# Luigi940260/orb-slam2-optimized

Hardware: AMD Instinct MI355X
Metric: RANSAC hypotheses/sec (EPnP relocalization batch, 2k corrs x 64 candidates) (higher is better)
Workload: dtype f64; 1 GPU; config 2 reloc_pnp: candidates x correspondences, iterate(300), exhaustive (40% inliers); candidates=64, candidates_per_gpu=64, correspondences=2000, hypotheses_per_candidate=300, params=SetRansacParameters(0.99,10,300,4,0.5,5.991)

## Files before the change

### orb-slam2-optimized_amd/csrc/kernels.hip

```cpp
#include <hip/hip_runtime.h>
#include <climits>

#ifndef RSC_REFINE_STAMPS
#define RSC_REFINE_STAMPS 0
#endif
namespace rsc {
__device__ uint64_t g_refine_stamps[64][24];
}
#ifndef RSC_SOLVE_STAMPS
#define RSC_SOLVE_STAMPS 0
#endif
namespace rsc {
__device__ uint64_t g_solve_stamps[3][4096][8];
}
#if RSC_SOLVE_STAMPS
#define RSC_JSVD_STAMP(k, j)                                                                           \
    do {                                                                                               \
        if (blockIdx.x < 4096 && (threadIdx.x & 63) == 0 && blockDim.x == 64) {                       \
            ::rsc::g_solve_stamps[2][blockIdx.x][j] = wall_clock64();                                  \
            ::rsc::g_solve_stamps[2][blockIdx.x][3] = (k);                                             \
        }                                                                                              \
    } while (0)
#define RSC_SOLVE_STAMP(st, k)                                                                         \
    do {                                                                                               \
// ... 12 lines not shown
#include "rsc_quad.h"
#include "rsc_math.h"
#include "rsc_kernels.h"

namespace rsc {

template <int NS>
__global__ __launch_bounds__(64) void pnp_eig_group_kernel(const DevPnP* __restrict__ probs,
                                                          const LaunchProb* __restrict__ lps,
                                                          const int2* __restrict__ wg_table,
                                                          const uint32_t* __restrict__ rng_T,
                                                          double* __restrict__ stage, int32_t* __restrict__ samples) {
    __shared__ __attribute__((aligned(16))) double smem[kEigHyps * kQuadRegion];
    pnp_eig_group_body<NS, 99, kEigLanes, kEigHyps>(probs, lps, wg_table, rng_T, stage, samples, smem);
}

template <int NS>
__global__ __launch_bounds__(128 * kSplitUnits) __attribute__((amdgpu_waves_per_eu(2))) void pnp_eig_split_kernel(
    const DevPnP* __restrict__ probs, const LaunchProb* __restrict__ lps, const int2* __restrict__ wg_table,
    int nwg_table, const uint32_t* __restrict__ rng_T, double* __restrict__ stage, int32_t* __restrict__ samples,
    unsigned* fault) {
    __shared__ __attribute__((aligned(16))) double smem[kSplitHyps * kQuadRegion];
    __shared__ __attribute__((aligned(16))) double dsub[kSplitHyps * kSplitDsub];
    __shared__ int pub[kSplitUnits], ack[kSplitUnits];
    pnp_eig_split_body<NS>(probs, lps, wg_table, nwg_table, rng_T, stage, samples, smem, dsub, pub, ack, fault);
}

template <int NS>
__global__ __launch_bounds__(64) void pnp_betas_kernel(const DevPnP* __restrict__ probs,
                                                       const LaunchProb* __restrict__ lps,
                                                       const int2* __restrict__ wg_table, int ngroups,
                                                       const double* __restrict__ stage,
                                                       const int32_t* __restrict__ samples,
                                                       float* __restrict__ poses, double* __restrict__ berr,
                                                       float* __restrict__ bpose, unsigned* __restrict__ bctr,
                                                       size_t hcap, int hb) {
    __shared__ __attribute__((aligned(16))) double smem[kBetasWaveSmemDoubles];
    pnp_betas_wave_body<NS>(probs, lps, wg_table, ngroups, hb, stage, samples, poses, berr, bpose, bctr, hcap, smem);
}

typedef float rsc_f2 __attribute__((ext_vector_type(2)));
__device__ __forceinline__ void pnp_inlier2(const float (&R)[9], const float (&t)[3], double fx, double fy, double cx,
                                            double cy, rsc_f2 X, rsc_f2 Y, rsc_f2 Z, rsc_f2 u, rsc_f2 v, rsc_f2 maxErr,
                                            bool& in0, bool& in1, bool& ok) {
    const rsc_f2 Xc = (R[0] * X + (R[1] * Y + R[2] * Z)) + t[0];
    const rsc_f2 Yc = (R[3] * X + (R[4] * Y + R[5] * Z)) + t[1];
    const rsc_f2 Zc = (R[6] * X + (R[7] * Y + R[8] * Z)) + t[2];
    const rsc_f2 r0 = {__builtin_amdgcn_rcpf(Zc.x), __builtin_amdgcn_rcpf(Zc.y)};
    const rsc_f2 e = __builtin_elementwise_fma(-Zc, r0, (rsc_f2){1.0f, 1.0f});
    const rsc_f2 iz = __builtin_elementwise_fma(e, r0, r0);
    const float a0 = fabsf(Zc.x), a1 = fabsf(Zc.y);
    ok = ok & (a0 >= 0x1p-126f) & (a0 <= 0x1p125f) & (a1 >= 0x1p-126f) & (a1 <= 0x1p125f);
    const rsc_f2 ue = {(float)(cx + fx * (double)Xc.x * (double)iz.x), (float)(cx + fx * (double)Xc.y * (double)iz.y)};
    const rsc_f2 ve = {(float)(cy + fy * (double)Yc.x * (double)iz.x), (float)(cy + fy * (double)Yc.y * (double)iz.y)};
    const rsc_f2 du = ue - u, dv = ve - v;
    const rsc_f2 e2 = du * du + dv * dv;
    in0 = e2.x < maxErr.x;
    in1 = e2.y < maxErr.y;
}

template <int PPT>
__global__ __launch_bounds__(256) void pnp_scan_kernel(const DevPnP* __restrict__ probs,
                                                       const LaunchProb* __restrict__ lps,
                                                       const int4* __restrict__ wg_table,
                                                       const float* __restrict__ poses,
                                                       int32_t* __restrict__ counts,
                                                       int32_t* __restrict__ counts_dev,
                                                       uint64_t* __restrict__ masks, int mask_words,
                                                       int32_t* __restrict__ qual) {
    constexpr int B = PPT <= 8 ? 64 : 512 / PPT;
    __shared__ int wave_cnt[4][B];
    __shared__ uint64_t mbuf[B][4][PPT];
    const int tid = threadIdx.x, lane = tid & 63, wave = tid >> 6;
    const int4 wt = wg_table[blockIdx.x];
    const LaunchProb& lp = lps[wt.x];
    const DevPnP& P = probs[lp.prob];
    const double fx = P.fx, fy = P.fy, cx = P.cx, cy = P.cy;
    float X[PPT], Y[PPT], Z[PPT], U[PPT], V[PPT], E[PPT];
    RSC_UNROLL for (int s = 0; s < PPT; ++s) {
        const int i = s * 256 + tid;
        if (i < P.n) {
            const float4 p = P.pts[i];
            const float2 q = P.uv[i];
            X[s] = p.x; Y[s] = p.y; Z[s] = p.z; E[s] = p.w * P.th2; U[s] = q.x; V[s] = q.y;
        } else {
            X[s] = 0.f; Y[s] = 0.f; Z[s] = 1.f; E[s] = -1.f; U[s] = 0.f; V[s] = 0.f;
        }
    }
    const float* pp = poses + (size_t)(lp.out0 + wt.y) * 12;
    float Rn[9], tn[3];
    RSC_UNROLL for (int k = 0; k < 9; ++k) Rn[k] = pp[k];
    RSC_UNROLL for (int k = 0; k < 3; ++k) tn[k] = pp[9 + k];
    for (int j = 0; j < wt.z; ++j) {
        float R[9], t[3];
        RSC_UNROLL for (int k = 0; k < 9; ++k) R[k] = Rn[k];
        RSC_UNROLL for (int k = 0; k < 3; ++k) t[k] = tn[k];
        if (j + 1 < wt.z) {
            pp += 12;
            RSC_UNROLL for (int k = 0; k < 9; ++k) Rn[k] = pp[k];
            RSC_UNROLL for (int k = 0; k < 3; ++k) tn[k] = pp[9 + k];
        }
        uint64_t b[PPT];
        if constexpr (PPT >= 2) {
            bool ok = true;
            RSC_UNROLL for (int s = 0; s < PPT; s += 2) {
                bool i0, i1;
                pnp_inlier2(R, t, fx, fy, cx, cy, (rsc_f2){X[s], X[s + 1]}, (rsc_f2){Y[s], Y[s + 1]},
                            (rsc_f2){Z[s], Z[s + 1]}, (rsc_f2){U[s], U[s + 1]}, (rsc_f2){V[s], V[s + 1]},
                            (rsc_f2){E[s], E[s + 1]}, i0, i1, ok);
                b[s] = __ballot(i0);
                b[s + 1] = __ballot(i1);
            }
            if (__builtin_expect(__any(!ok), 0)) {
                RSC_UNROLL for (int s = 0; s < PPT; ++s)
                    b[s] = __ballot(pnp_inlier(R, t, fx, fy, cx, cy, X[s], Y[s], Z[s], U[s], V[s], E[s]));
            }
        } else {
            RSC_UNROLL for (int s = 0; s < PPT; ++s)
                b[s] = __ballot(pnp_inlier(R, t, fx, fy, cx, cy, X[s], Y[s], Z[s], U[s], V[s], E[s]));
        }
        int cnt = 0;
        uint64_t mine = 0;
        RSC_UNROLL for (int s = 0; s < PPT; ++s) {
            cnt += __popcll(b[s]);
            mine = (lane == s) ? b[s] : mine;
        }
        const int jb = j % B;
        if (lane < PPT) mbuf[jb][wave][lane] = mine;
        if (lane == 0) wave_cnt[wave][jb] = cnt;
        if (jb == B - 1 || j == wt.z - 1) {
            __syncthreads();
// ... 758 lines not shown
    if (count <= 0) return hipSuccess;
    sim3_pick_kernel<<<count, 256, 0, st>>>(lps, counts, poses, pick);
    return hipGetLastError();
}

hipError_t launch_gather_records(const float* src, int stride, int take, const int32_t* idx, int n, float* dst,
                                 hipStream_t st) {
    if (n <= 0) return hipSuccess;
    gather_records_kernel<<<(n * take + 255) / 256, 256, 0, st>>>(src, stride, take, idx, n, dst);
    return hipGetLastError();
}

__global__ void rng_stream_kernel(const uint32_t* __restrict__ T, Window31 w, int g0, int n, int32_t* __restrict__ out) {
    const int i = blockIdx.x * blockDim.x + threadIdx.x;
    if (i >= n) return;
    uint32_t ww[31];
    RSC_UNROLL for (int j = 0; j < 31; ++j) ww[j] = w.w[j];
    out[i] = (int32_t)(rng_word(T, ww, g0 + i) >> 1);
}

template <int N>
static hipError_t launch_eig_rows(int nwgE, const int2* wgtE, const DevPnP* probs, const LaunchProb* lps,
                                  const uint32_t* T, double* stage, int32_t* samples, hipStream_t st) {
    if constexpr (kEigHyps == 4 * kRowsGroups) {
        pnp_eig_rows_kernel<N><<<nwgE, 256, 0, st>>>(probs, lps, wgtE, T, stage, samples);
        return hipSuccess;
    } else {
        return hipErrorInvalidValue;
    }
}

hipError_t launch_pnp_solve_split(int ns, int nwgE, const int2* wgtE, int nwgB, const int2* wgtB,
                                  const DevPnP* probs, const LaunchProb* lps, const uint32_t* T, double* stage,
                                  float* poses, int32_t* samples, const BetasScratch& bs, hipStream_t st,
                                  hipEvent_t eig_begin, hipEvent_t eig_end, bool eig_rows, bool eig_split,
                                  unsigned* fault, int betas_hb) {
    if (ns < 4 || ns > 6 || betas_hb < 1 || betas_hb > kBetasHyps) return hipErrorInvalidValue;
    if (eig_split && !eig_rows && !fault) return hipErrorInvalidValue;
    if (eig_begin) (void)hipEventRecord(eig_begin, st);
    switch (ns) {
#define RSC_CASE(N)                                                                                   \
    case N:                                                                                           \
        if (eig_rows) {                                                                               \
            const hipError_t e = launch_eig_rows<N>(nwgE, wgtE, probs, lps, T, stage, samples, st);   \
            if (e != hipSuccess) return e;                                                            \
        } else if (eig_split)                                                                         \
            pnp_eig_split_kernel<N><<<(nwgE + kSplitUnits - 1) / kSplitUnits, 128 * kSplitUnits, 0, st>>>( \
                probs, lps, wgtE, nwgE, T, stage, samples, fault);                                    \
        else                                                                                          \
            pnp_eig_group_kernel<N><<<nwgE, 64, 0, st>>>(probs, lps, wgtE, T, stage, samples);        \
        if (eig_end) (void)hipEventRecord(eig_end, st);                                               \
        pnp_betas_kernel<N><<<3 * nwgB, 64, 0, st>>>(probs, lps, wgtB, nwgB, stage, samples, poses,   \
                                                     bs.err, bs.pose, bs.ctr, bs.hcap, betas_hb);     \
        break;
        RSC_CASE(4) RSC_CASE(5) RSC_CASE(6)
#undef RSC_CASE
        default: return hipErrorInvalidValue;
    }
    return hipGetLastError();
}

__global__ __launch_bounds__(256) void selftest_math_kernel(int fn, const double* __restrict__ x, int n,
                                                            double* __restrict__ out) {
    const int i = blockIdx.x * 256 + threadIdx.x;
    if (i >= n) return;
    const double v = x[i];
    double r;
    switch (fn) {
        case 0: r = dm::sin(v); break;
        case 1: r = dm::cos(v); break;
        case 2: r = dm::acos(v); break;
        case 3: r = dm::cbrt(v); break;
        case 4: r = dm::log(v); break;
        case 5: r = (double)dm::logf((float)v); break;
        case 6: r = sqrt_unit(v); break;
        case 7: r = recip_unit(v); break;
        case 11: r = dm::pow_1_3(v); break;
        case 12: r = dm::pow_3_2(v); break;
        case 13: {
            const float z = (float)v;
            const float r0 = __builtin_amdgcn_rcpf(z);
            r = (double)__builtin_fmaf(__builtin_fmaf(-z, r0, 1.0f), r0, r0);
            break;
        }

        default: {
// ... 52 lines not shown
    copy_bytes_kernel<<<blocks, 256, 0, st>>>(static_cast<const uint8_t*>(src), static_cast<uint8_t*>(dst), n, unit);
    return hipGetLastError();
}

__global__ __launch_bounds__(64) void signal_kernel(uint32_t* flag, uint32_t v) {
    if (threadIdx.x == 0) __hip_atomic_store(flag, v, __ATOMIC_RELEASE, __HIP_MEMORY_SCOPE_SYSTEM);
}

hipError_t launch_signal(uint32_t* host_flag, uint32_t value, hipStream_t st) {
    signal_kernel<<<1, 64, 0, st>>>(host_flag, value);
    return hipGetLastError();
}

hipError_t launch_upload16(const void* host_src, void* dev_dst, size_t n16, hipStream_t st) {
    if (n16 == 0) return hipSuccess;
    const unsigned blocks = (unsigned)((n16 + 255) / 256);
    upload16_kernel<<<blocks, 256, 0, st>>>(static_cast<const uint4*>(host_src), static_cast<uint4*>(dev_dst), n16);
    return hipGetLastError();
}

hipError_t launch_selftest_math(int fn, const double* x, int n, double* out, hipStream_t st) {
    if (fn < 0 || fn > 13 || n <= 0) return hipErrorInvalidValue;
    if (fn == 10) {
        if (n % 34) return hipErrorInvalidValue;
        const int nrec = n / 34;
        selftest_qr_kernel<<<(nrec + 255) / 256, 256, 0, st>>>(x, nrec, out);
        return hipGetLastError();
    }
    selftest_math_kernel<<<(n + 255) / 256, 256, 0, st>>>(fn, x, n, out);
    return hipGetLastError();
}

hipError_t launch_pnp_scan(int ppt, int nwg, const DevPnP* probs, const LaunchProb* lps, const int4* wgt,
                           const float* poses, int32_t* counts, int32_t* counts_dev, uint64_t* masks, int mask_words,
                           int32_t* qual, hipStream_t st) {
    switch (ppt) {
#define RSC_CASE(P) case P: pnp_scan_kernel<P><<<nwg, 256, 0, st>>>(probs, lps, wgt, poses, counts, counts_dev, masks, mask_words, qual); break;
        RSC_CASE(1) RSC_CASE(2) RSC_CASE(4) RSC_CASE(8) RSC_CASE(16) RSC_CASE(32)
#undef RSC_CASE
        default: return hipErrorInvalidValue;
    }
    return hipGetLastError();
}

hipError_t read_solve_stamps(uint64_t* out) {
    return hipMemcpyFromSymbol(out, HIP_SYMBOL(g_solve_stamps), sizeof(uint64_t) * 3 * 4096 * 8, 0, hipMemcpyDeviceToHost);
}

hipError_t read_refine_stamps(uint64_t* out) {
    return hipMemcpyFromSymbol(out, HIP_SYMBOL(g_refine_stamps), sizeof(uint64_t) * 64 * 24, 0, hipMemcpyDeviceToHost);
}

hipError_t launch_pnp_refine(int njobs, const DevPnP* probs, const RefineJob* jobs, unsigned* fault, hipStream_t st) {
    if (!fault) return hipErrorInvalidValue;
    pnp_refine_kernel<<<njobs, 256, 0, st>>>(probs, jobs, fault);
    return hipGetLastError();
}

hipError_t launch_pnp_select_refine(int nsel, const DevPnP* probs, const RefineSel* sels, const int32_t* counts,
                                    uint64_t* masks, int mask_words, const float* poses, RefineSelOut* out,
                                    unsigned* fault, hipStream_t st) {
    if (nsel <= 0) return hipSuccess;
    if (!fault) return hipErrorInvalidValue;
    pnp_select_refine_kernel<<<nsel, 256, 0, st>>>(probs, sels, counts, masks, mask_words, poses, out, fault);
    return hipGetLastError();
}

hipError_t launch_sim3_solve(int nwg, const DevSim3* probs, const LaunchProb* lps, const int2* wgt, const uint32_t* T,
                             float* poses, int32_t* samples, hipStream_t st) {
    sim3_solve_kernel<<<nwg, 64, 0, st>>>(probs, lps, wgt, T, poses, samples);
    return hipGetLastError();
}

hipError_t launch_sim3_scan(int ppt, int nwg, const DevSim3* probs, const LaunchProb* lps, const int4* wgt,
                            const float* poses, int32_t* counts, int32_t* counts_dev, uint64_t* masks, int mask_words,
// ... 19 lines not shown
```

### orb-slam2-optimized_amd/csrc/rsc_api.cpp

```cpp
#include <hip/hip_runtime.h>
#include <cstdio>
#include <cstdlib>
#include <algorithm>
#include <array>
#include <chrono>
#include <cmath>
#include <cstring>
#include <string>
#include <vector>
#include <memory>
#include "../../include/rsc.h"
#include "rsc_kernels.h"
#include "rsc_engine.h"
#include "rsc_poseopt.h"
#include "rsc_sim3opt.h"
#include "rsc_orbmatch.h"
#include "rsc_sim3match.h"
#include "rsc_frameproj.h"
#include "rsc_kfproj.h"
#include "rsc_localproj.h"
#include "rsc_sim3compose.h"
#include "rsc_kfdb.h"
#include "rsc_bowvoc.h"

// ... 73 lines not shown
    rb.clear();
    for (size_t i = 0; i < n; ++i)
        if (i == 0 || prob_of(src[i]) != prob_of(src[i - 1])) rb.push_back(i);
    rb.push_back(n);
    size_t left[X] = {};
    for (int x = 0; x < X; ++x) runs[x].clear();
    for (size_t r = 0; r + 1 < rb.size(); ++r) {
        int best = 0;
        for (int x = 1; x < X; ++x) if (left[x] < left[best]) best = x;
        runs[best].push_back((int)r);
        left[best] += rb[r + 1] - rb[r];
    }
    size_t cr[X] = {}, cp[X] = {};
    for (size_t b = 0; b < n; ++b) {
        int x = (int)(b % X);
        if (!left[x])
            for (int y = 0; y < X; ++y) if (left[y] > left[x]) x = y;
        const int r = runs[x][cr[x]];
        wgs[b] = src[rb[r] + cp[x]];
        if (++cp[x] == rb[r + 1] - rb[r]) { cp[x] = 0; ++cr[x]; }
        --left[x];
    }
}

int scan_chunk(int total_hyps) {
    static const int target = [] {
        const char* m = std::getenv("RSC_SCAN_WGS");
        return m ? std::max(1, std::atoi(m)) : 2048;
    }();
    int hc = 32;
    while (hc > 8 && (total_hyps + hc - 1) / hc < target) hc >>= 1;
    return hc;
}

int ppt_for(int n) {
    int need = (n + 255) / 256;
    int p = 1;
    while (p < need) p <<= 1;
    return p;
}

}

constexpr int kSoCoopCUs = 256;
constexpr int kFaultWord = 4;

struct rsc_context {
    int device = 0;
    hipStream_t stream = nullptr;
    bool own_stream = false;
    RngTable table;
    DevBuf<uint32_t> d_table;
    DevBuf<float> d_poses;
    DevBuf<int32_t> d_counts;
    DevBuf<uint64_t> d_masks;
    DevBuf<int32_t> d_samples;
    DevBuf<double> d_stage;
    DevBuf<double> d_berr;
    DevBuf<float> d_bpose;
    DevBuf<unsigned> d_bctr;
    DevBuf<float> d_gather;
    DevBuf<double> d_mposes;
    DevBuf<char> d_desc;
    PinBuf<char> h_desc;
    PinBuf<int32_t> h_counts;
    PinBuf<int32_t> h_qual;
    DevBuf<char> d_pnp_tab;
    std::vector<int> pnp_tab_key;
    size_t pnp_tab_quad[3] = {0, 0, 0}, pnp_tab_solve[3] = {0, 0, 0}, pnp_tab_scan = 0;
    PinBuf<float> h_small;
    PinBuf<float> h_pick;
    DevBuf<char> d_refine;
    DevBuf<RefineSelOut> d_selout;
    PinBuf<RefineSelOut> h_selout;
    DevBuf<char> d_po_in;
    DevBuf<char> d_so_in;
    PinBuf<char> h_so_in;
    DevBuf<char> d_so_res;
    PinBuf<char> h_so_res;
    DevBuf<char> d_po_res;
    PinBuf<char> h_po_in;
    PinBuf<char> h_po_res;
    DevBuf<char> d_s3m;
    PinBuf<char> h_s3m;
    struct S3mPair { size_t o_m1, o_m2; int n1, n2; };
    std::vector<S3mPair> s3m_last;
    DevBuf<char> d_bow;
    PinBuf<char> h_bow;
    DevBuf<char> d_fp;
    PinBuf<char> h_fp;
    int mask_words = 0;
    bool keep_samples = true;
    bool timing = false;
    hipEvent_t ev[12] = {};
    double last_ms[6] = {0, 0, 0, 0, 0, 0};
    double host_us[4] = {0, 0, 0, 0};
    bool direct_counts = true;
    bool fused_refine = true;
    bool dma_upload = false;
    int eig_rows_max_wgs = kEigRowsDefaultWgs;
    int betas_small_hb = kBetasHyps;
    bool eig_split = true;
// ... 211 lines not shown
            total += H[i];
            maxN = std::max(maxN, S[i]->N);
        }
        const int ppt = ppt_for(maxN);
        if (ppt > 32) {
            g_last_error = "more than 8192 correspondences per problem";
            return RSC_ERR_UNSUPPORTED;
        }
        const int mw = ppt * 4;
        C->mask_words = mw;
        fused_count = 0;
        const bool fused = C->fused_refine && total <= kFusedRefineMaxHyps;
        thread_local std::vector<RefineSel> sels_tl;
        std::vector<RefineSel>& sels = sels_tl;
        sels.resize(fused ? count : 0);
        for (int i = 0; fused && i < count; ++i) {
            rsc_pnp* p = of(S[i]);
            RefineSel& r = sels[i];
            r.prob = i;
            r.out0 = lps[i].out0;
            r.H = H[i];
            r.min_inliers = S[i]->mRansacMinInliers;
            r.best0 = S[i]->mnBestInliers;
            r.rows0 = S[i]->max_rows;
            r.best = p->d_best;
            r.refined = p->d_refined;
            r.words = p->words;
        }
        thread_local std::vector<int2> solve_wgs_tl[3], quad_wgs_tl[3];
        thread_local std::vector<int4> scan_wgs_tl;
        std::vector<int2>* solve_wgs = solve_wgs_tl;
        std::vector<int2>* quad_wgs = quad_wgs_tl;
        std::vector<int4>& scan_wgs = scan_wgs_tl;
        const int HC = scan_chunk(total);
        const int hb = (total <= kEigHyps * C->eig_rows_max_wgs) ? C->betas_small_hb : kBetasHyps;

        thread_local std::vector<int> shape_tl;
        std::vector<int>& shape = shape_tl;
        thread_local std::vector<int> key_tl;
        std::vector<int>& key = key_tl;
        key.clear();
        key.push_back(count);
        key.push_back(HC);
        key.push_back(hb);
        for (int i = 0; i < count; ++i) {
            key.push_back(S[i]->mRansacMinSet);
            key.push_back(H[i]);
        }
        if (key != shape) {
            for (int g = 0; g < 3; ++g) { solve_wgs[g].clear(); quad_wgs[g].clear(); }
            scan_wgs.clear();
            for (int i = 0; i < count; ++i) {
                const int g = S[i]->mRansacMinSet - 4;
                for (int h0 = 0; h0 < H[i]; h0 += hb) solve_wgs[g].push_back(make_int2(i, h0));
                for (int h0 = 0; h0 < H[i]; h0 += kEigHyps) quad_wgs[g].push_back(make_int2(i, h0));
                for (int h0 = 0; h0 < H[i]; h0 += HC)
                    scan_wgs.push_back(make_int4(i, h0, std::min(HC, H[i] - h0), 0));
            }
            for (int g = 0; g < 3; ++g) {
                xcd_order(solve_wgs[g], [](const int2& w) { return w.x; });
                xcd_order(quad_wgs[g], [](const int2& w) { return w.x; });
            }
            xcd_order(scan_wgs, [](const int4& w) { return w.x; });
            shape.assign(key.begin(), key.end());
        }
        if (C->pnp_tab_key != key || !C->d_pnp_tab.p) {
            std::vector<char> tab;
            auto put = [&](const void* p, size_t n) {
                const size_t o = tab.size();
                tab.resize(o + ((n + 15) & ~(size_t)15));
                if (n) std::memcpy(tab.data() + o, p, n);
                return o;
            };
            for (int g = 0; g < 3; ++g) C->pnp_tab_solve[g] = put(solve_wgs[g].data(), solve_wgs[g].size() * sizeof(int2));
            for (int g = 0; g < 3; ++g) C->pnp_tab_quad[g] = put(quad_wgs[g].data(), quad_wgs[g].size() * sizeof(int2));
            C->pnp_tab_scan = put(scan_wgs.data(), scan_wgs.size() * sizeof(int4));
            C->pnp_tab_key.clear();
            if (int e = C->d_pnp_tab.ensure(std::max(tab.size(), (size_t)16))) return e;
            RSC_HIP(hipMemcpyAsync(C->d_pnp_tab.p, tab.data(), tab.size(), hipMemcpyHostToDevice, C->stream));
            RSC_HIP(hipStreamSynchronize(C->stream));
            C->pnp_tab_key = key;
        }
        Blob b;
        const size_t o_probs = b.add(probs.data(), probs.size() * sizeof(DevPnP));
        const size_t o_lps = b.add(lps.data(), lps.size() * sizeof(LaunchProb));
        const size_t o_sel = fused ? b.add(sels.data(), sels.size() * sizeof(RefineSel)) : 0;
        if (int e = upload_blob(C, b)) return e;
        const char* tab = C->d_pnp_tab.p;
        if (int e = C->d_poses.ensure((size_t)total * 12)) return e;
        int32_t* cnt_dst = nullptr;
        if (int e = counts_target(C, total, &cnt_dst)) return e;
        if (int e = C->h_qual.ensure((size_t)count)) return e;
        std::memset(C->h_qual.p, 0, (size_t)count * sizeof(int32_t));
        int32_t* cnt_dev = nullptr;
        if (fused) {
            if (C->direct_counts) {
                if (int e = C->d_counts.ensure((size_t)total)) return e;
                cnt_dev = C->d_counts.p;
            }
            if (int e = C->d_selout.ensure((size_t)count)) return e;
            if (int e = C->h_selout.ensure((size_t)count)) return e;
        }
        if (int e = C->d_masks.ensure((size_t)total * mw)) return e;
        if (int e = C->d_samples.ensure((size_t)total * 8)) return e;
        if (int e = C->d_stage.ensure((size_t)total * kStageDoubles)) return e;
        if (int e = C->d_berr.ensure((size_t)total * 3)) return e;
        if (int e = C->d_bpose.ensure((size_t)total * 36)) return e;
        size_t groups = 0;
        for (int g = 0; g < 3; ++g) groups = std::max(groups, solve_wgs[g].size());
        const size_t had = C->d_bctr.cap;
        if (int e = C->d_bctr.ensure(groups)) return e;
        if (C->d_bctr.cap != had) RSC_HIP(hipMemsetAsync(C->d_bctr.p, 0, C->d_bctr.cap * sizeof(unsigned), C->stream));
        const BetasScratch bs{C->d_berr.p, C->d_bpose.p, C->d_bctr.p, (size_t)total};
        const char* base = C->d_desc.p;
        const DevPnP* dprobs = reinterpret_cast<const DevPnP*>(base + o_probs);
        const LaunchProb* dlps = reinterpret_cast<const LaunchProb*>(base + o_lps);
        host_mark(C, 0);
        timing_begin(C, 0);
        bool first_group = true;
        for (int g = 0; g < 3; ++g) {
            if (solve_wgs[g].empty()) continue;
            hipEvent_t eb = (C->timing && !first_group) ? C->ev[6 + 2 * g] : nullptr;
            RSC_HIP(launch_pnp_solve_split(4 + g, (int)quad_wgs[g].size(),
                                          reinterpret_cast<const int2*>(tab + C->pnp_tab_quad[g]), (int)solve_wgs[g].size(),
                                          reinterpret_cast<const int2*>(tab + C->pnp_tab_solve[g]), dprobs, dlps,
                                          C->d_table.p, C->d_stage.p, C->d_poses.p, C->d_samples.p, bs, C->stream,
                                          eb, C->timing ? C->ev[7 + 2 * g] : nullptr,
                                          (int)quad_wgs[g].size() <= C->eig_rows_max_wgs, C->eig_split,
                                          C->h_flag + kFaultWord, hb));
            first_group = false;
        }
        timing_begin(C, 1);
        RSC_HIP(launch_pnp_scan(ppt, (int)scan_wgs.size(), dprobs, dlps, reinterpret_cast<const int4*>(tab + C->pnp_tab_scan),
                                C->d_poses.p, cnt_dst, cnt_dev, C->d_masks.p, mw, C->h_qual.p, C->stream));
        timing_begin(C, 2);
        if (fused) {
            timing_begin(C, 3);
            RSC_HIP(launch_pnp_select_refine(count, dprobs, reinterpret_cast<const RefineSel*>(base + o_sel),
                                             cnt_dev ? cnt_dev : cnt_dst, C->d_masks.p, mw, C->d_poses.p,
                                             C->d_selout.p, C->h_flag + kFaultWord, C->stream));
            timing_begin(C, 4);
            RSC_HIP(hipMemcpyAsync(C->h_selout.p, C->d_selout.p, sizeof(RefineSelOut) * count, hipMemcpyDeviceToHost,
                                   C->stream));
        }
        if (!C->direct_counts)
            RSC_HIP(hipMemcpyAsync(C->h_counts.p, C->d_counts.p, (size_t)total * 4, hipMemcpyDeviceToHost, C->stream));
        host_mark(C, 1);
        if (int e = stream_wait(C)) return e;
        host_mark(C, 2);
        if (int e = take_fault(C)) return e;
        if (C->timing) {
            float a = 0, s = 0;
            (void)hipEventElapsedTime(&a, C->ev[0], C->ev[1]);
            (void)hipEventElapsedTime(&s, C->ev[1], C->ev[2]);
            C->last_ms[0] += a;
            C->last_ms[1] += s;
            C->last_ms[3] += 1;
            C->last_ms[4] += total;
            bool first = true;
            for (int g = 0; g < 3; ++g) {
                if (solve_wgs[g].empty()) continue;
                float e = 0;
                (void)hipEventElapsedTime(&e, first ? C->ev[0] : C->ev[6 + 2 * g], C->ev[7 + 2 * g]);
                C->last_ms[5] += e;
                first = false;
            }
            if (fused) {
// ... 3917 lines not shown
```

### orb-slam2-optimized_amd/csrc/rsc_kernels.h

```cpp
#pragma once
#include <cstdint>
#include <hip/hip_runtime.h>

namespace rsc {

struct DevPnP {
    const float4* pts;
    const float2* uv;
    int n;
    float fx, fy, cx, cy;
    float th2;
    int rows;
    double* pws;
    double* us;
    double* als;
};

struct DevSim3 {
    const float4* x1;
    const float4* x2;
    const float4* pim;
    int n;
    float K1[4], K2[4];
};
// ... 47 lines not shown
    int k;
    int adopt;
    int rows_after;
    int count;
    float pose[12];
    float best_pose[12];
};

struct Window31 {
    uint32_t w[31];
};
constexpr int kMlQuadHyps = 16;
hipError_t launch_mlpnp_solve(int ns, bool cov, int nwg, const DevML* probs, const LaunchProb* lps, const int2* wgt,
                              const uint32_t* T, double* poses, int32_t* samples, hipStream_t st);
hipError_t launch_mlpnp_scan(int ppt, int nwg, const DevML* probs, const LaunchProb* lps, const int4* wgt,
                             const double* poses, int32_t* counts, uint64_t* masks, int mask_words, hipStream_t st);
hipError_t launch_selftest_math(int fn, const double* x, int n, double* out, hipStream_t st);
hipError_t launch_upload16(const void* host_src, void* dev_dst, size_t n16, hipStream_t st);
hipError_t launch_signal(uint32_t* host_flag, uint32_t value, hipStream_t st);
hipError_t launch_copy_bytes(const void* src, void* dst, size_t n, hipStream_t st);
hipError_t launch_gather_records(const float* src, int stride, int take, const int32_t* idx, int n, float* dst,
                                 hipStream_t st);
hipError_t launch_rng_stream(const uint32_t* T, const uint32_t* window, int g0, int n, int32_t* out, hipStream_t st);

constexpr int kEigLanes = 2;
#ifndef RSC_EIG_HYPS
#define RSC_EIG_HYPS 20
#endif
constexpr int kEigHyps = RSC_EIG_HYPS;
constexpr int kStageDoubles = 48 + 24 + 12;
struct BetasScratch {
    double* err;
    float* pose;
    unsigned* ctr;
    size_t hcap;
};
#ifndef RSC_BETAS_HYPS
#define RSC_BETAS_HYPS 64
#endif
constexpr int kBetasHyps = RSC_BETAS_HYPS;
constexpr int kEigRowsDefaultWgs = 64;
hipError_t launch_pnp_solve_split(int ns, int nwgE, const int2* wgtE, int nwgB, const int2* wgtB,
                                  const DevPnP* probs, const LaunchProb* lps, const uint32_t* T, double* stage,
                                  float* poses, int32_t* samples, const BetasScratch& bs, hipStream_t st,
                                  hipEvent_t eig_begin = nullptr, hipEvent_t eig_end = nullptr, bool eig_rows = false,
                                  bool eig_split = false, unsigned* fault = nullptr, int betas_hb = kBetasHyps);
hipError_t launch_pnp_scan(int ppt, int nwg, const DevPnP* probs, const LaunchProb* lps, const int4* wgt,
                           const float* poses, int32_t* counts, int32_t* counts_dev, uint64_t* masks, int mask_words,
                           int32_t* qual, hipStream_t st);
hipError_t launch_pnp_select_refine(int nsel, const DevPnP* probs, const RefineSel* sels, const int32_t* counts,
                                    uint64_t* masks, int mask_words, const float* poses, RefineSelOut* out,
                                    unsigned* fault, hipStream_t st);
constexpr int kFusedRefineMaxHyps = 4096;
hipError_t read_refine_stamps(uint64_t* out);
hipError_t read_solve_stamps(uint64_t* out);
hipError_t read_ml_stamps(uint64_t* out);
hipError_t launch_pnp_refine(int njobs, const DevPnP* probs, const RefineJob* jobs, unsigned* fault, hipStream_t st);
hipError_t launch_sim3_solve(int nwg, const DevSim3* probs, const LaunchProb* lps, const int2* wgt,
                             const uint32_t* T, float* poses, int32_t* samples, hipStream_t st);
hipError_t launch_sim3_scan(int ppt, int nwg, const DevSim3* probs, const LaunchProb* lps, const int4* wgt,
                            const float* poses, int32_t* counts, int32_t* counts_dev, uint64_t* masks, int mask_words,
                            hipStream_t st);
hipError_t launch_sim3_pick(int count, const LaunchProb* lps, const int32_t* counts, const float* poses,
                            float* pick, hipStream_t st);

}
```

### orb-slam2-optimized_amd/csrc/rsc_quad.h

```cpp
#pragma once
#include "rsc_core.h"
#include "rsc_epnp.h"
#include "rsc_kernels.h"

#ifndef RSC_EIG_PHASE
#define RSC_EIG_PHASE(k) \
    do {                 \
    } while (0)
#endif
#ifndef RSC_SOLVE_STAMP
#define RSC_SOLVE_STAMP(st, k) \
    do {                       \
    } while (0)
#endif

namespace rsc {

constexpr int kQuadT = 144;
constexpr int kQuadE = 55;
constexpr int kQuadRegion = kQuadT + kQuadE + 1;
constexpr int kStEv = 0, kStAl = 48, kStCws = 72;
constexpr int kBetasWaveSmemDoubles = 66 * kBetasHyps;

RSC_HD constexpr int quad_eoff(int i) { return 10 * i - (i * (i - 1)) / 2; }
// ... 837 lines not shown
    RSC_SPLIT_STAMP(6);
    if (lane == 0) {
        const int steps = __hip_atomic_load(pub + unit, __ATOMIC_RELAXED, __HIP_MEMORY_SCOPE_WORKGROUP);
        __hip_atomic_store(pub + unit, steps | kSplitDone, __ATOMIC_RELEASE, __HIP_MEMORY_SCOPE_WORKGROUP);
    }
    RSC_SPLIT_STAMP(4);
#undef RSC_SPLIT_STAMP
}

struct StageEvView {
    const double* evp;
    double* Lp;
    RSC_HD double ev(int r, int c) const { return evp[r * 4 + c]; }
    RSC_HD double& L(int i, int j) const { return Lp[(i * 10 + j) * kBetasHyps]; }
    RSC_HD double& rho(int i) const { return Lp[(60 + i) * kBetasHyps]; }
};

RSC_HD void betas_block(int b, int ngroups, int& g, int& apx) {
    const int q = ngroups / 8;
    if (b < 24 * q) {
        g = (b % 8) + 8 * (b / 24);
        apx = (b / 8) % 3;
    } else {
        const int r = ngroups - 8 * q, rem = b - 24 * q;
        g = 8 * q + rem % r;
        apx = rem / r;
    }
}

template <int NS>
__device__ __forceinline__ void pnp_betas_wave_body(const DevPnP* __restrict__ probs, const LaunchProb* __restrict__ lps,
                                                    const int2* __restrict__ wg_table, int ngroups, int hb,
                                                    const double* __restrict__ stage,
                                                    const int32_t* __restrict__ samples, float* __restrict__ poses,
                                                    double* __restrict__ berr, float* __restrict__ bpose,
                                                    unsigned* __restrict__ bctr, size_t hcap, double* smem) {
    const int lane = threadIdx.x;
    int g, apx;
    betas_block(blockIdx.x, ngroups, g, apx);
    const int2 wt = wg_table[g];
    const LaunchProb& lp = lps[wt.x];
    const bool active = lane < hb && wt.y + lane < lp.H;
    const int hm = wt.y + lane % hb;
    const int h = active ? wt.y + lane : (hm < lp.H ? hm : wt.y);
    const DevPnP& P = probs[lp.prob];
    const size_t rec = (size_t)(lp.out0 + h);
    const double* in = stage + rec * kStageDoubles;
    const StageEvView V{in + kStEv, smem + lane % kBetasHyps};
    RSC_SOLVE_STAMP(1, 0);
    compute_L_6x10(V);
    {
        double cws[4][3];
        RSC_UNROLL for (int i = 0; i < 4; ++i)
            RSC_UNROLL for (int c = 0; c < 3; ++c) cws[i][c] = in[kStCws + i * 3 + c];
        auto d2 = [&](int a, int b) {
            double x = cws[a][0] - cws[b][0], y = cws[a][1] - cws[b][1], z = cws[a][2] - cws[b][2];
            return ered3(x * x, y * y, z * z);
        };
        V.rho(0) = d2(0, 1); V.rho(1) = d2(0, 2); V.rho(2) = d2(0, 3);
        V.rho(3) = d2(1, 2); V.rho(4) = d2(1, 3); V.rho(5) = d2(2, 3);
    }
    double betas[4] = {0.0, 0.0, 0.0, 0.0};
    RSC_SOLVE_STAMP(1, 1);
    if (apx == 0) find_betas<1>(V, betas);
    else if (apx == 1) find_betas<2>(V, betas);
    else find_betas<3>(V, betas);
    RSC_SOLVE_STAMP(1, 2);
    gauss_newton(V, betas);
    RSC_SOLVE_STAMP(1, 3);
    HypStore<NS> st;
    RSC_UNROLL for (int i = 0; i < NS; ++i) {
        const int id = samples[rec * 8 + i];
        const float4 p = P.pts[id];
        const float2 uv = P.uv[id];
        st.pw_[i][0] = p.x; st.pw_[i][1] = p.y; st.pw_[i][2] = p.z;
        st.u_[i][0] = uv.x; st.u_[i][1] = uv.y;
        RSC_UNROLL for (int j = 0; j < 4; ++j) st.al_[i][j] = in[kStAl + i * 4 + j];
    }
    st.rows_ = P.rows;
    st.spw = P.pws;
    st.sal = P.als;
    const Intrinsics K{(double)P.fx, (double)P.fy, (double)P.cx, (double)P.cy};
    const double pw0[3] = {in[kStCws + 0], in[kStCws + 1], in[kStCws + 2]};
    double R[3][3], t[3];
    RSC_SOLVE_STAMP(1, 4);
    const double err = compute_R_and_t(st, K, V, betas, pw0, R, t);
    RSC_SOLVE_STAMP(1, 5);
    float pz[12];
    RSC_UNROLL for (int r = 0; r < 3; ++r)
        RSC_UNROLL for (int c = 0; c < 3; ++c) pz[3 * r + c] = (float)R[r][c];
    RSC_UNROLL for (int r = 0; r < 3; ++r) pz[9 + r] = (float)t[r];
    if (active) {
        berr[apx * hcap + rec] = err;
        RSC_UNROLL for (int k = 0; k < 12; ++k) bpose[(apx * 12 + k) * hcap + rec] = pz[k];
    }
    asm volatile("s_waitcnt vmcnt(0)" ::: "memory");
    __builtin_amdgcn_fence(__ATOMIC_RELEASE, "agent");
    asm volatile("s_waitcnt vmcnt(0)" ::: "memory");
    unsigned prev = 0;
    if (lane == 0) prev = __hip_atomic_fetch_add(bctr + g, 1u, __ATOMIC_RELAXED, __HIP_MEMORY_SCOPE_AGENT);
    prev = __builtin_amdgcn_readlane(prev, 0);
    RSC_SOLVE_STAMP(1, 6);
#if RSC_SOLVE_STAMPS
    if ((threadIdx.x & 63) == 0 && blockIdx.x < 4096) g_solve_stamps[1][blockIdx.x][7] = (uint64_t)apx | ((uint64_t)g << 8);
#endif
    if (prev != 2) return;
    __builtin_amdgcn_fence(__ATOMIC_ACQUIRE, "agent");
    asm volatile("s_waitcnt vmcnt(0)" ::: "memory");
    if (lane == 0) __hip_atomic_store(bctr + g, 0u, __ATOMIC_RELAXED, __HIP_MEMORY_SCOPE_AGENT);
    if (!active) return;
    double e[3];
    RSC_UNROLL for (int a = 0; a < 3; ++a) e[a] = (a == apx) ? err : berr[a * hcap + rec];
    int best = 0;
    double be = e[0];
    if (e[1] < be) { be = e[1]; best = 1; }
    if (e[2] < be) { be = e[2]; best = 2; }
    float* o = poses + rec * 12;
    if (best == apx) {
        RSC_UNROLL for (int k = 0; k < 12; ++k) o[k] = pz[k];
    } else {
        RSC_UNROLL for (int k = 0; k < 12; ++k) o[k] = bpose[(best * 12 + k) * hcap + rec];
    }
}

}
```

Before: 73.64 million hypotheses/s.

## Move best-of-three pose selection into scan kernel and size scan chunks by occupancy

The betas kernel no longer chains its three approximation blocks through an atomic counter with release/acquire fences. It now writes each error and pose (as float4 stores in a per-hypothesis layout) to scratch. The scan kernel reads the three errors per hypothesis, picks the best with ballots, and writes the chosen pose to the poses buffer while it uses it for inlier counting. Separately, the host now splits scan work into per-candidate chunks based on the kernel's occupancy capacity rather than a fixed chunk size. The trade is extra global reads in the scan kernel, and the chunk sizes it picks must stay at or below one wave's width.

```diff
diff --git a/orb-slam2-optimized_amd/csrc/kernels.hip b/orb-slam2-optimized_amd/csrc/kernels.hip
--- a/orb-slam2-optimized_amd/csrc/kernels.hip
+++ b/orb-slam2-optimized_amd/csrc/kernels.hip
@@ -68,11 +68,10 @@
                                                        const int2* __restrict__ wg_table, int ngroups,
                                                        const double* __restrict__ stage,
                                                        const int32_t* __restrict__ samples,
-                                                       float* __restrict__ poses, double* __restrict__ berr,
-                                                       float* __restrict__ bpose, unsigned* __restrict__ bctr,
+                                                       double* __restrict__ berr, float* __restrict__ bpose,
                                                        size_t hcap, int hb) {
     __shared__ __attribute__((aligned(16))) double smem[kBetasWaveSmemDoubles];
-    pnp_betas_wave_body<NS>(probs, lps, wg_table, ngroups, hb, stage, samples, poses, berr, bpose, bctr, hcap, smem);
+    pnp_betas_wave_body<NS>(probs, lps, wg_table, ngroups, hb, stage, samples, berr, bpose, hcap, smem);
 }
 
 typedef float rsc_f2 __attribute__((ext_vector_type(2)));
@@ -99,7 +98,9 @@
 __global__ __launch_bounds__(256) void pnp_scan_kernel(const DevPnP* __restrict__ probs,
                                                        const LaunchProb* __restrict__ lps,
                                                        const int4* __restrict__ wg_table,
-                                                       const float* __restrict__ poses,
+                                                       const double* __restrict__ berr,
+                                                       const float* __restrict__ bpose, size_t hcap,
+                                                       float* __restrict__ poses,
                                                        int32_t* __restrict__ counts,
                                                        int32_t* __restrict__ counts_dev,
                                                        uint64_t* __restrict__ masks, int mask_words,
@@ -112,6 +113,13 @@
     const LaunchProb& lp = lps[wt.x];
     const DevPnP& P = probs[lp.prob];
     const double fx = P.fx, fy = P.fy, cx = P.cx, cy = P.cy;
+    const size_t rec0 = (size_t)(lp.out0 + wt.y);
+    double e0 = 0.0, e1 = 0.0, e2 = 0.0;
+    if (lane < wt.z) {
+        e0 = berr[rec0 + lane];
+        e1 = berr[hcap + rec0 + lane];
+        e2 = berr[2 * hcap + rec0 + lane];
+    }
     float X[PPT], Y[PPT], Z[PPT], U[PPT], V[PPT], E[PPT];
     RSC_UNROLL for (int s = 0; s < PPT; ++s) {
         const int i = s * 256 + tid;
@@ -123,7 +131,22 @@
             X[s] = 0.f; Y[s] = 0.f; Z[s] = 1.f; E[s] = -1.f; U[s] = 0.f; V[s] = 0.f;
         }
     }
-    const float* pp = poses + (size_t)(lp.out0 + wt.y) * 12;
+    int best = 0;
+    {
+        double be = e0;
+        if (e1 < be) { be = e1; best = 1; }
+        if (e2 < be) { be = e2; best = 2; }
+    }
+    const uint64_t pick1 = __ballot(best == 1), pick2 = __ballot(best == 2);
+    auto pose_of = [&](int j) {
+        const size_t apx = (size_t)((pick1 >> j) & 1u) + 2 * (size_t)((pick2 >> j) & 1u);
+        return bpose + (apx * hcap + rec0 + (size_t)j) * 12;
+    };
+    for (int w = tid; w < wt.z * 12; w += 256) {
+        const int hj = w / 12, k = w - 12 * hj;
+        poses[(rec0 + hj) * 12 + k] = pose_of(hj)[k];
+    }
+    const float* pp = pose_of(0);
     float Rn[9], tn[3];
     RSC_UNROLL for (int k = 0; k < 9; ++k) Rn[k] = pp[k];
     RSC_UNROLL for (int k = 0; k < 3; ++k) tn[k] = pp[9 + k];
@@ -132,7 +155,7 @@
         RSC_UNROLL for (int k = 0; k < 9; ++k) R[k] = Rn[k];
         RSC_UNROLL for (int k = 0; k < 3; ++k) t[k] = tn[k];
         if (j + 1 < wt.z) {
-            pp += 12;
+            pp = pose_of(j + 1);
             RSC_UNROLL for (int k = 0; k < 9; ++k) Rn[k] = pp[k];
             RSC_UNROLL for (int k = 0; k < 3; ++k) tn[k] = pp[9 + k];
         }
@@ -957,7 +980,7 @@
 
 hipError_t launch_pnp_solve_split(int ns, int nwgE, const int2* wgtE, int nwgB, const int2* wgtB,
                                   const DevPnP* probs, const LaunchProb* lps, const uint32_t* T, double* stage,
-                                  float* poses, int32_t* samples, const BetasScratch& bs, hipStream_t st,
+                                  int32_t* samples, const BetasScratch& bs, hipStream_t st,
                                   hipEvent_t eig_begin, hipEvent_t eig_end, bool eig_rows, bool eig_split,
                                   unsigned* fault, int betas_hb) {
     if (ns < 4 || ns > 6 || betas_hb < 1 || betas_hb > kBetasHyps) return hipErrorInvalidValue;
@@ -975,8 +998,8 @@
         else                                                                                          \
             pnp_eig_group_kernel<N><<<nwgE, 64, 0, st>>>(probs, lps, wgtE, T, stage, samples);        \
         if (eig_end) (void)hipEventRecord(eig_end, st);                                               \
-        pnp_betas_kernel<N><<<3 * nwgB, 64, 0, st>>>(probs, lps, wgtB, nwgB, stage, samples, poses,   \
-                                                     bs.err, bs.pose, bs.ctr, bs.hcap, betas_hb);     \
+        pnp_betas_kernel<N><<<3 * nwgB, 64, 0, st>>>(probs, lps, wgtB, nwgB, stage, samples,          \
+                                                     bs.err, bs.pose, bs.hcap, betas_hb);             \
         break;
         RSC_CASE(4) RSC_CASE(5) RSC_CASE(6)
 #undef RSC_CASE
@@ -1095,15 +1118,24 @@
 }
 
 hipError_t launch_pnp_scan(int ppt, int nwg, const DevPnP* probs, const LaunchProb* lps, const int4* wgt,
-                           const float* poses, int32_t* counts, int32_t* counts_dev, uint64_t* masks, int mask_words,
-                           int32_t* qual, hipStream_t st) {
+                           const BetasScratch& bs, float* poses, int32_t* counts, int32_t* counts_dev, uint64_t* masks,
+                           int mask_words, int32_t* qual, hipStream_t st) {
     switch (ppt) {
-#define RSC_CASE(P) case P: pnp_scan_kernel<P><<<nwg, 256, 0, st>>>(probs, lps, wgt, poses, counts, counts_dev, masks, mask_words, qual); break;
+#define RSC_CASE(P) case P: pnp_scan_kernel<P><<<nwg, 256, 0, st>>>(probs, lps, wgt, bs.err, bs.pose, bs.hcap, poses, counts, counts_dev, masks, mask_words, qual); break;
         RSC_CASE(1) RSC_CASE(2) RSC_CASE(4) RSC_CASE(8) RSC_CASE(16) RSC_CASE(32)
 #undef RSC_CASE
         default: return hipErrorInvalidValue;
     }
     return hipGetLastError();
+}
+
+hipError_t pnp_scan_occupancy(int ppt, int* wgs_per_cu) {
+    switch (ppt) {
+#define RSC_CASE(P) case P: return hipOccupancyMaxActiveBlocksPerMultiprocessor(wgs_per_cu, reinterpret_cast<const void*>(&pnp_scan_kernel<P>), 256, 0);
+        RSC_CASE(1) RSC_CASE(2) RSC_CASE(4) RSC_CASE(8) RSC_CASE(16) RSC_CASE(32)
+#undef RSC_CASE
+        default: return hipErrorInvalidValue;
+    }
 }
 
 hipError_t read_solve_stamps(uint64_t* out) {
diff --git a/orb-slam2-optimized_amd/csrc/rsc_api.cpp b/orb-slam2-optimized_amd/csrc/rsc_api.cpp
--- a/orb-slam2-optimized_amd/csrc/rsc_api.cpp
+++ b/orb-slam2-optimized_amd/csrc/rsc_api.cpp
@@ -129,6 +129,37 @@
     while (hc > 8 && (total_hyps + hc - 1) / hc < target) hc >>= 1;
     return hc;
 }
+bool scan_wgs_overridden() {
+    static const bool set = std::getenv("RSC_SCAN_WGS") != nullptr;
+    return set;
+}
+
+constexpr int kScanMinChunk = 8;
+void pnp_scan_partition(const int* H, int count, int capacity, int batch, std::vector<int>& chunks) {
+    chunks.assign((size_t)count, 1);
+    int64_t total = 0;
+    for (int i = 0; i < count; ++i) total += H[i];
+    if (total <= 0) return;
+    capacity = std::max(capacity, 1);
+    batch = std::max(batch, kScanMinChunk);
+    const int kmax = (int)(total / capacity) + 1;
+    for (int k = 1; k <= kmax; ++k) {
+        bool fits = true;
+        for (int i = 0; i < count; ++i) {
+            const int h = std::max(H[i], 1);
+            const int lo = (h + batch - 1) / batch, hi = (h + kScanMinChunk - 1) / kScanMinChunk;
+            const int64_t share = (int64_t)k * capacity * h / total;
+            if (share < lo && k < kmax) { fits = false; break; }
+            chunks[i] = (int)std::min<int64_t>(std::max<int64_t>(share, lo), hi);
+        }
+        if (fits) break;
+    }
+}
+inline void even_chunk(int H, int n, int c, int& h0, int& len) {
+    const int q = H / n, r = H % n;
+    h0 = c * q + std::min(c, r);
+    len = q + (c < r ? 1 : 0);
+}
 
 int ppt_for(int n) {
     int need = (n + 255) / 256;
@@ -155,7 +186,6 @@
     DevBuf<double> d_stage;
     DevBuf<double> d_berr;
     DevBuf<float> d_bpose;
-    DevBuf<unsigned> d_bctr;
     DevBuf<float> d_gather;
     DevBuf<double> d_mposes;
     DevBuf<char> d_desc;
@@ -165,6 +195,7 @@
     DevBuf<char> d_pnp_tab;
     std::vector<int> pnp_tab_key;
     size_t pnp_tab_quad[3] = {0, 0, 0}, pnp_tab_solve[3] = {0, 0, 0}, pnp_tab_scan = 0;
+    int pnp_scan_capacity[6] = {0, 0, 0, 0, 0, 0};
     PinBuf<float> h_small;
     PinBuf<float> h_pick;
     DevBuf<char> d_refine;
@@ -442,7 +473,24 @@
         std::vector<int2>* solve_wgs = solve_wgs_tl;
         std::vector<int2>* quad_wgs = quad_wgs_tl;
         std::vector<int4>& scan_wgs = scan_wgs_tl;
-        const int HC = scan_chunk(total);
+        const int HC = scan_wgs_overridden() ? scan_chunk(total) : 0;
+        int scan_cap = 0;
+        if (!HC) {
+            int lg = 0;
+            while ((1 << lg) < ppt) ++lg;
+            if (!C->pnp_scan_capacity[lg]) {
+                int per_cu = 0, cus = 0;
+                RSC_HIP(pnp_scan_occupancy(ppt, &per_cu));
+                RSC_HIP(hipDeviceGetAttribute(&cus, hipDeviceAttributeMultiprocessorCount, C->device));
+                if (per_cu <= 0 || cus <= 0) {
+                    g_last_error = "pnp_scan_kernel: no resident workgroup (occupancy query)";
+                    return RSC_ERR_INTERNAL;
+                }
+                C->pnp_scan_capacity[lg] = per_cu * cus;
+            }
+            scan_cap = C->pnp_scan_capacity[lg];
+        }
+        const int scan_batch = ppt <= 8 ? 64 : 512 / ppt;
         const int hb = (total <= kEigHyps * C->eig_rows_max_wgs) ? C->betas_small_hb : kBetasHyps;
 
         thread_local std::vector<int> shape_tl;
@@ -452,6 +500,8 @@
         key.clear();
         key.push_back(count);
         key.push_back(HC);
+        key.push_back(scan_cap);
+        key.push_back(scan_batch);
         key.push_back(hb);
         for (int i = 0; i < count; ++i) {
             key.push_back(S[i]->mRansacMinSet);
@@ -460,12 +510,23 @@
         if (key != shape) {
             for (int g = 0; g < 3; ++g) { solve_wgs[g].clear(); quad_wgs[g].clear(); }
             scan_wgs.clear();
+            thread_local std::vector<int> chunks_tl;
+            std::vector<int>& chunks = chunks_tl;
+            if (!HC) pnp_scan_partition(H, count, scan_cap, scan_batch, chunks);
             for (int i = 0; i < count; ++i) {
                 const int g = S[i]->mRansacMinSet - 4;
                 for (int h0 = 0; h0 < H[i]; h0 += hb) solve_wgs[g].push_back(make_int2(i, h0));
                 for (int h0 = 0; h0 < H[i]; h0 += kEigHyps) quad_wgs[g].push_back(make_int2(i, h0));
-                for (int h0 = 0; h0 < H[i]; h0 += HC)
-                    scan_wgs.push_back(make_int4(i, h0, std::min(HC, H[i] - h0), 0));
+                if (HC) {
+                    for (int h0 = 0; h0 < H[i]; h0 += HC)
+                        scan_wgs.push_back(make_int4(i, h0, std::min(HC, H[i] - h0), 0));
+                } else if (H[i] > 0) {
+                    for (int c = 0; c < chunks[i]; ++c) {
+                        int h0, len;
+                        even_chunk(H[i], chunks[i], c, h0, len);
+                        scan_wgs.push_back(make_int4(i, h0, len, 0));
+                    }
+                }
             }
             for (int g = 0; g < 3; ++g) {
                 xcd_order(solve_wgs[g], [](const int2& w) { return w.x; });
@@ -516,12 +577,7 @@
         if (int e = C->d_stage.ensure((size_t)total * kStageDoubles)) return e;
         if (int e = C->d_berr.ensure((size_t)total * 3)) return e;
         if (int e = C->d_bpose.ensure((size_t)total * 36)) return e;
-        size_t groups = 0;
-        for (int g = 0; g < 3; ++g) groups = std::max(groups, solve_wgs[g].size());
-        const size_t had = C->d_bctr.cap;
-        if (int e = C->d_bctr.ensure(groups)) return e;
-        if (C->d_bctr.cap != had) RSC_HIP(hipMemsetAsync(C->d_bctr.p, 0, C->d_bctr.cap * sizeof(unsigned), C->stream));
-        const BetasScratch bs{C->d_berr.p, C->d_bpose.p, C->d_bctr.p, (size_t)total};
+        const BetasScratch bs{C->d_berr.p, C->d_bpose.p, (size_t)total};
         const char* base = C->d_desc.p;
         const DevPnP* dprobs = reinterpret_cast<const DevPnP*>(base + o_probs);
         const LaunchProb* dlps = reinterpret_cast<const LaunchProb*>(base + o_lps);
@@ -534,7 +590,7 @@
             RSC_HIP(launch_pnp_solve_split(4 + g, (int)quad_wgs[g].size(),
                                           reinterpret_cast<const int2*>(tab + C->pnp_tab_quad[g]), (int)solve_wgs[g].size(),
                                           reinterpret_cast<const int2*>(tab + C->pnp_tab_solve[g]), dprobs, dlps,
-                                          C->d_table.p, C->d_stage.p, C->d_poses.p, C->d_samples.p, bs, C->stream,
+                                          C->d_table.p, C->d_stage.p, C->d_samples.p, bs, C->stream,
                                           eb, C->timing ? C->ev[7 + 2 * g] : nullptr,
                                           (int)quad_wgs[g].size() <= C->eig_rows_max_wgs, C->eig_split,
                                           C->h_flag + kFaultWord, hb));
@@ -542,7 +598,7 @@
         }
         timing_begin(C, 1);
         RSC_HIP(launch_pnp_scan(ppt, (int)scan_wgs.size(), dprobs, dlps, reinterpret_cast<const int4*>(tab + C->pnp_tab_scan),
-                                C->d_poses.p, cnt_dst, cnt_dev, C->d_masks.p, mw, C->h_qual.p, C->stream));
+                                bs, C->d_poses.p, cnt_dst, cnt_dev, C->d_masks.p, mw, C->h_qual.p, C->stream));
         timing_begin(C, 2);
         if (fused) {
             timing_begin(C, 3);
diff --git a/orb-slam2-optimized_amd/csrc/rsc_kernels.h b/orb-slam2-optimized_amd/csrc/rsc_kernels.h
--- a/orb-slam2-optimized_amd/csrc/rsc_kernels.h
+++ b/orb-slam2-optimized_amd/csrc/rsc_kernels.h
@@ -103,7 +103,6 @@
 struct BetasScratch {
     double* err;
     float* pose;
-    unsigned* ctr;
     size_t hcap;
 };
 #ifndef RSC_BETAS_HYPS
@@ -113,12 +112,13 @@
 constexpr int kEigRowsDefaultWgs = 64;
 hipError_t launch_pnp_solve_split(int ns, int nwgE, const int2* wgtE, int nwgB, const int2* wgtB,
                                   const DevPnP* probs, const LaunchProb* lps, const uint32_t* T, double* stage,
-                                  float* poses, int32_t* samples, const BetasScratch& bs, hipStream_t st,
+                                  int32_t* samples, const BetasScratch& bs, hipStream_t st,
                                   hipEvent_t eig_begin = nullptr, hipEvent_t eig_end = nullptr, bool eig_rows = false,
                                   bool eig_split = false, unsigned* fault = nullptr, int betas_hb = kBetasHyps);
 hipError_t launch_pnp_scan(int ppt, int nwg, const DevPnP* probs, const LaunchProb* lps, const int4* wgt,
-                           const float* poses, int32_t* counts, int32_t* counts_dev, uint64_t* masks, int mask_words,
-                           int32_t* qual, hipStream_t st);
+                           const BetasScratch& bs, float* poses, int32_t* counts, int32_t* counts_dev, uint64_t* masks,
+                           int mask_words, int32_t* qual, hipStream_t st);
+hipError_t pnp_scan_occupancy(int ppt, int* wgs_per_cu);
 hipError_t launch_pnp_select_refine(int nsel, const DevPnP* probs, const RefineSel* sels, const int32_t* counts,
                                     uint64_t* masks, int mask_words, const float* poses, RefineSelOut* out,
                                     unsigned* fault, hipStream_t st);
diff --git a/orb-slam2-optimized_amd/csrc/rsc_quad.h b/orb-slam2-optimized_amd/csrc/rsc_quad.h
--- a/orb-slam2-optimized_amd/csrc/rsc_quad.h
+++ b/orb-slam2-optimized_amd/csrc/rsc_quad.h
@@ -893,9 +893,9 @@
 __device__ __forceinline__ void pnp_betas_wave_body(const DevPnP* __restrict__ probs, const LaunchProb* __restrict__ lps,
                                                     const int2* __restrict__ wg_table, int ngroups, int hb,
                                                     const double* __restrict__ stage,
-                                                    const int32_t* __restrict__ samples, float* __restrict__ poses,
+                                                    const int32_t* __restrict__ samples,
                                                     double* __restrict__ berr, float* __restrict__ bpose,
-                                                    unsigned* __restrict__ bctr, size_t hcap, double* smem) {
+                                                    size_t hcap, double* smem) {
     const int lane = threadIdx.x;
     int g, apx;
     betas_block(blockIdx.x, ngroups, g, apx);
@@ -953,35 +953,13 @@
     RSC_UNROLL for (int r = 0; r < 3; ++r) pz[9 + r] = (float)t[r];
     if (active) {
         berr[apx * hcap + rec] = err;
-        RSC_UNROLL for (int k = 0; k < 12; ++k) bpose[(apx * 12 + k) * hcap + rec] = pz[k];
-    }
-    asm volatile("s_waitcnt vmcnt(0)" ::: "memory");
-    __builtin_amdgcn_fence(__ATOMIC_RELEASE, "agent");
-    asm volatile("s_waitcnt vmcnt(0)" ::: "memory");
-    unsigned prev = 0;
-    if (lane == 0) prev = __hip_atomic_fetch_add(bctr + g, 1u, __ATOMIC_RELAXED, __HIP_MEMORY_SCOPE_AGENT);
-    prev = __builtin_amdgcn_readlane(prev, 0);
+        float4* o = reinterpret_cast<float4*>(bpose + (apx * hcap + rec) * 12);
+        RSC_UNROLL for (int k = 0; k < 3; ++k) o[k] = make_float4(pz[4 * k], pz[4 * k + 1], pz[4 * k + 2], pz[4 * k + 3]);
+    }
     RSC_SOLVE_STAMP(1, 6);
 #if RSC_SOLVE_STAMPS
     if ((threadIdx.x & 63) == 0 && blockIdx.x < 4096) g_solve_stamps[1][blockIdx.x][7] = (uint64_t)apx | ((uint64_t)g << 8);
 #endif
-    if (prev != 2) return;
-    __builtin_amdgcn_fence(__ATOMIC_ACQUIRE, "agent");
-    asm volatile("s_waitcnt vmcnt(0)" ::: "memory");
-    if (lane == 0) __hip_atomic_store(bctr + g, 0u, __ATOMIC_RELAXED, __HIP_MEMORY_SCOPE_AGENT);
-    if (!active) return;
-    double e[3];
-    RSC_UNROLL for (int a = 0; a < 3; ++a) e[a] = (a == apx) ? err : berr[a * hcap + rec];
-    int best = 0;
-    double be = e[0];
-    if (e[1] < be) { be = e[1]; best = 1; }
-    if (e[2] < be) { be = e[2]; best = 2; }
-    float* o = poses + rec * 12;
-    if (best == apx) {
-        RSC_UNROLL for (int k = 0; k < 12; ++k) o[k] = pz[k];
-    } else {
-        RSC_UNROLL for (int k = 0; k < 12; ++k) o[k] = bpose[(best * 12 + k) * hcap + rec];
-    }
-}
-
-}
+}
+
+}
```

Measured after the change: 75.50 million hypotheses/s (median of 6 runs). +2.5%, better.
